# VSF1/foo_dsp_resampler

Hardware: AMD Instinct MI355X
Metric: Msamples/s, 44.1k->96k float32 'Best' (input channel-samples) (higher is better)
Workload: dtype f64; 1 GPU; BASELINE configs[1]: 44.1k->96k 2ch float32 Best; 256 independent 2-channel streams on this GPU, 481689 frames per push, device-resident in/out (RRX_flow_device); streams_per_gpu=256, frames_per_push=481689, channels=2, chain=dft->poly

## Files before the change

foo_dsp_resampler_amd/csrc/fused_fast.hip:

```cpp
#include "fft_device.hpp"
#include "fifo_device.hpp"
#include "kernels.hpp"

#include <algorithm>
#include <atomic>
#include <cstdlib>
#include <cstdio>
#include <type_traits>

namespace rsmp {

namespace {
typedef unsigned int rsmp_v2u __attribute__((ext_vector_type(2)));
typedef unsigned int rsmp_v4u __attribute__((ext_vector_type(4)));
template <typename E> struct Frame;
template <> struct Frame<float> {
  typedef float2 P;
  static __device__ __forceinline__ double in(float s) { return (double)s; }
  static __device__ __forceinline__ float out(double y) { return (float)y; }
};
template <> struct Frame<double> {
  typedef double2 P;
  static __device__ __forceinline__ double in(double s) { return s; }
  static __device__ __forceinline__ double out(double y) { return y; }
};
template <> struct Frame<short> {
  typedef short2 P;
  static __device__ __forceinline__ double in(short s) { return pcm_in(s); }
  static __device__ __forceinline__ short out(double y) { return pcm_out16(y); }
};
template <> struct Frame<int> {
  typedef int2 P;
  static __device__ __forceinline__ double in(int s) { return pcm_in(s); }
  static __device__ __forceinline__ int out(double y) { return pcm_out32(y); }
};
__device__ __forceinline__ double2 load_g(const double2 *p) { return *p; }
constexpr int kPad = 32;
constexpr int kSA = kFusedSA, kSB0 = kFusedSB0;
}

template <int LOG2P, int KS, bool OUT64, bool SPLIT, bool OGEN, bool TWO = false, typename E = float>
__device__ __forceinline__ void fused_fast_body(const FusedArgs &a, const FastIo &io)
{
  typedef Frame<E> Fr;
  typedef typename Fr::P E2;
  const E *const io_in = static_cast<const E *>(io.in), *const io_in_ring = static_cast<const E *>(io.in_ring);
  E *const io_out = static_cast<E *>(io.out), *const io_out_ring = static_cast<E *>(io.out_ring);
  static_assert(!TWO || SPLIT, "two rounds from registers: sub-blocked form only");
  static_assert(!SPLIT || LOG2P == 12, "sub-blocked form: 4096-point components");
  static_assert(!OGEN || (SPLIT && !OUT64), "generic float output exists for the sub-blocked form only");
  constexpr int LOG2N = 12, N = 1 << LOG2N, P = 1 << LOG2P;
  constexpr int T = N / 16, TF = P / 16;
  extern __shared__ __attribute__((aligned(16))) double lds[];

  const int tid = threadIdx.x;
  const int npairs = a.d.C >> 1;
  int bl, pair;
  if (!item_map(blockIdx.x, a.d.nblocks, npairs, a.d.hp, bl, pair)) return;
  const long long B = a.d.B0 + bl;
  const int hp = io.nch >> 1, strm = pair / hp, pin = pair - strm * hp;
  SubBlock sb = {0, 0, 0, 0};
  long long e0_split = 0;
  if constexpr (SPLIT) {
    const int kr = bl / a.d.nsub;
    sb = sub_block(bl - kr * a.d.nsub, a.d.V, a.d.Vs, a.d.Pref);
    e0_split = (a.d.Bref0 + kr) * a.d.q + sb.win;
  }
  const int V = SPLIT ? sb.len : a.d.V;
  const bool fwd_active = tid < TF;
  const double2 *__restrict__ Gp = a.d.G;
  double2 *smp = reinterpret_cast<double2 *>(lds) + kPad;
  const int nm1 = a.n - 1;

#ifdef RSMP_STAMPS_BUILD
  const bool stamping = a.stamps && (blockIdx.x & 63) == 5;
  unsigned long long tstamp = stamping ? __builtin_readcyclecounter() : 0;
#define RSMP_STAMP(slot)                                          \
  if (stamping) {                                                  \
    const unsigned long long now = __builtin_readcyclecounter();  \
    if (tid == 0) atomicAdd(a.stamps + (slot), now - tstamp);      \
    tstamp = now;                                                  \
  }
#else
#define RSMP_STAMP(slot)
#endif

  constexpr bool FWD8 = LOG2P == LOG2N - 1;
  constexpr int NLD = FWD8 ? 8 : 16, TL = FWD8 ? T : TF;
  c64 v[16];
  c64 u8[8];
  c64 z0[SPLIT ? 16 : 1];
  double2 wf[FWD8 ? fft8_tw_regs(LOG2P) : 1];
  if constexpr (FWD8) fft8_tw_load<LOG2P>(wf, tid, a.d.tw_fwd8);
  {
    const long long e0 = SPLIT ? e0_split : B * a.d.q;
    const bool ld_active = FWD8 || fwd_active;
    if (SPLIT && io.in_unaligned) {
      const E *pe = io_in + strm * io.in_stream_stride + 2 * pin, *pr = io_in_ring + strm * io.in_ring_stream_stride + 2 * pin;
#pragma unroll
      for (int s = 0; s < NLD; ++s) {
        const long long e = e0 + tid + s * TL;
        const E *f = e >= io.in_abs0 ? pe + (e - io.in_abs0) * io.nch : pr + (e & io.in_ring_mask) * io.nch;
        v[s] = {Fr::in(f[0]), Fr::in(f[1])};
      }
    } else
    if (e0 >= io.in_abs0) {
      const E2 *p2 = reinterpret_cast<const E2 *>(io_in + strm * io.in_stream_stride + (e0 - io.in_abs0) * io.nch + 2 * pin);
      if (ld_active) {
#pragma unroll
        for (int s = 0; s < NLD; ++s) {
          const E2 f = p2[(unsigned)((tid + s * TL) * hp)];
          (FWD8 ? u8[s & 7] : v[s]) = {Fr::in(f.x), Fr::in(f.y)};
        }
      }
    } else if (ld_active) {
      const E *pe = io_in + strm * io.in_stream_stride + 2 * pin, *pr = io_in_ring + strm * io.in_ring_stream_stride + 2 * pin;
#pragma unroll
      for (int s = 0; s < NLD; ++s) {
        const long long e = e0 + tid + s * TL;
        const E2 f = *reinterpret_cast<const E2 *>(e >= io.in_abs0 ? pe + (e - io.in_abs0) * io.nch : pr + (e & io.in_ring_mask) * io.nch);
        (FWD8 ? u8[s & 7] : v[s]) = {Fr::in(f.x), Fr::in(f.y)};
      }
    }
  }
  RSMP_STAMP(0)
  if constexpr (FWD8) {
    double2 g[16];
    fft8_regs_pre<LOG2P, -1>(u8, tid, wf, lds, [&](int p) {
      if (p == 1) {
#pragma unroll
        for (int s = 0; s < 16; ++s) g[s] = load_g(Gp + (unsigned)(tid + s * T));
      }
    });
    RSMP_STAMP(1)
#pragma unroll
    for (int s = 0; s < 16; ++s) v[s] = cmul(u8[s & 7], c64{g[s].x, g[s].y});
    __syncthreads();
  } else {
  fft_regs<LOG2P, -1, LOG2P == LOG2N ? 2 : 0, kPfFwd>(v, tid, fwd_active, a.d.tw_fwd, lds);
  RSMP_STAMP(1)
  if constexpr (LOG2P < LOG2N) {
    double2 g[16];
#pragma unroll
    for (int s = 0; s < 16; ++s) g[s] = load_g(Gp + tid + s * T);
    double2 *l2 = reinterpret_cast<double2 *>(lds);
    if (fwd_active) {
#pragma unroll
      for (int u = 0; u < 8; ++u) l2[tid + u * TF] = make_double2(v[2 * u + 1].x, v[2 * u + 1].y);
    }
    __syncthreads();
    c64 z[8];
    if (fwd_active) {
#pragma unroll
      for (int u = 0; u < 8; ++u) z[u] = v[2 * u];
    } else {
#pragma unroll
      for (int u = 0; u < 8; ++u) {
        const double2 q = l2[tid - TF + u * TF];
        z[u] = {q.x, q.y};
      }
    }
#pragma unroll
    for (int s = 0; s < 16; ++s) v[s] = cmul(z[s & 7], c64{g[s].x, g[s].y});
    __syncthreads();
  } else if constexpr (SPLIT) {
    c64 xs[16];
#pragma unroll
    for (int s = 0; s < 16; ++s) {
      xs[s] = v[s];
      const double2 g = load_g(Gp + tid + s * T);
      v[s] = cmul(xs[s], c64{g.x, g.y});
    }
    fft_regs<LOG2N, +1, 2, kPfInv>(v, tid, true, a.d.tw_inv, lds);
    double2 g1[16];
#pragma unroll
    for (int s = 0; s < 16; ++s) g1[s] = load_g(Gp + N + tid + s * T);
#pragma unroll
    for (int s = 0; s < 16; ++s) {
      z0[s] = v[s];
      v[s] = cmul(xs[s], c64{g1[s].x, g1[s].y});
    }
    __syncthreads();
    fft_regs<LOG2N, +1, 2, kPfInv>(v, tid, true, a.d.tw_inv, lds);
  } else {
#pragma unroll
    for (int s = 0; s < 16; ++s) {
      const double2 g = load_g(Gp + tid + s * T);
      v[s] = cmul(v[s], c64{g.x, g.y});
    }
  }
  }
  RSMP_STAMP(2)
  if constexpr (!SPLIT) fft_regs<LOG2N, +1, 2, kPfInv>(v, tid, true, a.d.tw_inv, lds);
  RSMP_STAMP(3)

  const int ca = 2 * pair, cb = ca + 1;
  {
    const int slot = (int)(B & a.seam_mask);
    double *seamA = a.seam + ((long long)(slot * (a.d.C + 1) + ca) * 2) * 32;
    double *seamB = a.seam + ((long long)(slot * (a.d.C + 1) + cb) * 2) * 32;
    if constexpr (SPLIT && TWO) {
      __syncthreads();
#pragma unroll
      for (int s = 0; s <= kSplitSA; ++s) {
        const int n = 2 * (tid + s * T);
        if (n < V && (s < kSplitSA || tid < kPad / 2)) {
          smp[n] = make_double2(z0[s].x, z0[s].y);
          smp[n + 1] = make_double2(v[s].x, v[s].y);
        }
      }
      if (tid < kPad) {
        smp[tid - kPad] = make_double2(0.0, 0.0);
        if (V < kSplitRaEnd + kPad) smp[V + tid] = make_double2(0.0, 0.0);
      }
      (void)seamA; (void)seamB;
    } else if constexpr (SPLIT) {
      __syncthreads();
#pragma unroll
      for (int s = 0; s < 16; ++s) {
        const int n = 2 * (tid + s * T - sb.shift);
        if (n >= 0 && n < V) {
          smp[n] = make_double2(z0[s].x, z0[s].y);
          smp[n + 1] = make_double2(v[s].x, v[s].y);
        }
      }
      if (tid < kPad) {
        smp[tid - kPad] = make_double2(0.0, 0.0);
        smp[V + tid] = make_double2(0.0, 0.0);
      }
      (void)seamA; (void)seamB;
    } else {
#pragma unroll
    for (int s = 0; s <= kSA; ++s) {
      const int n = tid + s * T;
      const bool whole = (s + 1) * T <= V;
      if (s < kSA ? (whole || n < V) : (tid < kPad && n < V)) smp[n] = make_double2(v[s].x, v[s].y);
    }
    if (tid < nm1) {
      seamA[tid] = v[0].x;
      seamB[tid] = v[0].y;
    }
    if (tid < kPad) {
      smp[tid - kPad] = make_double2(0.0, 0.0);
      if (V < kSA * T + kPad) smp[V + tid] = make_double2(0.0, 0.0);
    }
    }
  }
  __syncthreads();
  if constexpr (SPLIT) {
    if (tid < nm1) {
      const int slot = (int)(B & a.seam_mask);
      const double2 t = smp[tid];
      a.seam[((long long)(slot * (a.d.C + 1) + ca) * 2) * 32 + tid] = t.x;
      a.seam[((long long)(slot * (a.d.C + 1) + cb) * 2) * 32 + tid] = t.y;
    }
  }
  const int tail0 = V - nm1;
  auto store_tail = [&](const double2 *img, int n0) {
    if (tid < nm1) {
      const int slot = (int)(B & a.seam_mask);
      const double2 t = img[tail0 + tid - n0];
      a.seam[((long long)(slot * (a.d.C + 1) + ca) * 2 + 1) * 32 + tid] = t.x;
      a.seam[((long long)(slot * (a.d.C + 1) + cb) * 2 + 1) * 32 + tid] = t.y;
    }
  };
  const bool tail_in_b = TWO ? tail0 >= kSplitRbStart : (!SPLIT && tail0 >= kSB0 * T);
  if (!tail_in_b) store_tail(smp, 0);
  RSMP_STAMP(4)

  const FusedBlock fb = a.blk[bl];
  const int lane = tid & 63, wave = __builtin_amdgcn_readfirstlane(tid >> 6);
  const int hi = lane >> 4, bq = (lane >> 2) & 3, jq = lane & 3;
  const int pl = a.polyL, step = a.step;
  const int frame_bytes = io.nch * (int)sizeof(E);
  char *const obytes = (OUT64 || OGEN) ? nullptr
                            : reinterpret_cast<char *>(io_out + strm * io.out_stream_stride + (a.out_offset2 + fb.i_lo - io.out_abs0) * io.nch + 2 * pin);
  const long long oabs0 = a.out_offset2 + fb.i_lo;
  E *const oext = OGEN ? io_out + strm * io.out_stream_stride + 2 * pin : nullptr;
  E *const oring = OGEN ? io_out_ring + strm * io.out_ring_stream_stride + 2 * pin : nullptr;
  const unsigned o64 = OUT64 ? (unsigned)((a.out_offset2 + fb.i_lo) & io.out64_mask) : 0u;
  const unsigned m64 = (unsigned)io.out64_mask;
  __amdgpu_buffer_rsrc_t orsrcA, orsrcB;
  if constexpr (OUT64) {
    double *ra = io.out64 + (long long)(2 * pair) * io.out64_chan_stride;
    orsrcA = __builtin_amdgcn_make_buffer_rsrc(ra, 0, (int)((io.out64_mask + 1) * 8), 0x00020000);
    orsrcB = __builtin_amdgcn_make_buffer_rsrc(ra + io.out64_chan_stride, 0, (int)((io.out64_mask + 1) * 8), 0x00020000);
  }
  const int rloc = 4 * bq + hi;
  const int ngrp = a.NGRP;
  const double2 *const cfm_lane = a.cfm2 + lane;
  const int *const qtab_lane = a.qtab + bq;

  const FusedWalk fw = fused_walk(fb, ngrp);
  auto poly_round = [&](int kb, int ke, const double2 *xs, int li_lo, int li_hi) {
    if (ke <= kb) return;
    const WalkRound wr = walk_round(fw, fb.K, kb, ke, ngrp);
    const int t0 = (wr.nt * wave) >> 2, t1 = (wr.nt * (wave + 1)) >> 2;
    if (t0 >= t1) return;
    int g, pc;
    walk_seek(wr, t0, g, pc);
    g = __builtin_amdgcn_readfirstlane(g);
    int p0 = __builtin_amdgcn_readfirstlane(walk_p0(fw, g));
    pc = __builtin_amdgcn_readfirstlane(4 * pc + p0);
    int pend = __builtin_amdgcn_readfirstlane(p0 + 4 * walk_ncs(fw, fb.K, kb, ke, g));
    const int lane_li = walk_lane_li(fb, kb, hi, jq, step);
    const int lane_ib = walk_lane_ib(fb, kb, jq, rloc, pl);
    const int cnt = walk_round_cnt(fb, fw, ke, pl);
    const __amdgpu_buffer_rsrc_t orsrc =
        __builtin_amdgcn_make_buffer_rsrc(obytes, 0, (!OUT64 && !OGEN && cnt > 0) ? (cnt - 1) * frame_bytes + 2 * (int)sizeof(E) : 0, 0x00020000);
    const int lane_off0 = __mul24(lane_ib, frame_bytes);
    const bool lane_dead_last = 16 * (ngrp - 1) + rloc >= pl;

    double cc[KS], cn[KS];
    double qcd = 0.0, qnd = 0.0;
    int qci = 0, qni = 0;
    auto load_tile = [&](int gg, double (&c_)[KS], double &qd_, int &qi_) {
      constexpr int KSP = (KS + 1) / 2;
      const double2 *cp = cfm_lane + gg * (KSP * 64);
#pragma unroll
      for (int s2 = 0; s2 < KSP; ++s2) {
        const double2 d = cp[s2 * 64];
        c_[2 * s2] = d.x;
        if (2 * s2 + 1 < KS) c_[2 * s2 + 1] = d.y;
        else qd_ = d.y;
      }
      if (!(KS & 1)) qi_ = qtab_lane[gg * 4];
    };
    auto qof = [&](double qd_, int qi_) { return (KS & 1) ? (int)qd_ : qi_; };
    load_tile(g, cc, qcd, qci);
    load_tile(min(g + 1, ngrp - 1), cn, qnd, qni);

    double2 x0[KS], x1[KS];
    auto fill = [&](double2 (&x)[KS], int q, int pstep) {
      const int li = max(li_lo, min(li_hi, q + pstep * step));
      const double2 *xp = xs + li;
#pragma unroll
      for (int s = 0; s < KS; ++s) x[s] = xp[4 * s];
    };
    int qc = qof(qcd, qci) + lane_li;
    fill(x0, qc, pc);

    int left = t1 - t0;
    auto tile = [&](const double2 (&xc)[KS], double2 (&xn)[KS]) {
      int wrap;
      asm("s_lshr_b32 %0, %1, 31" : "=s"(wrap) : "s"(pend - 8 - pc));
      const int gnext = g + wrap;
      int pnext = pc + 4, pend_next = pend;
      if (wrap != 0 && left > 1) {
        if constexpr (KS & 1) asm volatile("v_cvt_i32_f64 %0, %1" : "=v"(qc) : "v"(qnd));
        else asm volatile("v_mov_b32 %0, %1" : "=v"(qc) : "v"(qni));
        qc += lane_li;
        if (gnext == wr.b1 || gnext == wr.b2) {
          p0 = __builtin_amdgcn_readfirstlane(walk_p0(fw, gnext));
          pend_next = __builtin_amdgcn_readfirstlane(p0 + 4 * walk_ncs(fw, fb.K, kb, ke, gnext));
        }
        pnext = p0;
      }
      fill(xn, qc, left > 1 ? pnext : pc);
      double accA = 0.0, accB = 0.0;
#pragma unroll
      for (int s = 0; s < KS; ++s) {
        accA = __builtin_amdgcn_mfma_f64_4x4x4f64(cc[s], xc[s].x, accA, 0, 0, 0);
        accB = __builtin_amdgcn_mfma_f64_4x4x4f64(cc[s], xc[s].y, accB, 0, 0, 0);
      }
      (void)x0;
      const int ib = lane_ib + 16 * g + pc * pl;
      if constexpr (OGEN) {
        if ((unsigned)ib < (unsigned)cnt && 16 * g + rloc < pl) {
          const long long A = oabs0 + ib;
          E *const p = (A >= io.out_abs0 && A < io.out_end) ? oext + (A - io.out_abs0) * io.nch : oring + (A & io.out_ring_mask) * io.nch;
          if (io.out_unaligned) {
            p[0] = Fr::out(accA);
            p[1] = Fr::out(accB);
          } else
            *reinterpret_cast<E2 *>(p) = E2{Fr::out(accA), Fr::out(accB)};
        }
      } else if constexpr (OUT64) {
        const bool ok = (unsigned)ib < (unsigned)cnt && 16 * g + rloc < pl;
        const unsigned off = ok ? ((o64 + (unsigned)ib) & m64) * 8u : 0xffffffffu;
        const rsmp_v2u da = {(unsigned)__double2loint(accA), (unsigned)__double2hiint(accA)};
        const rsmp_v2u db = {(unsigned)__double2loint(accB), (unsigned)__double2hiint(accB)};
        __builtin_amdgcn_raw_buffer_store_b64(da, orsrcA, (int)off, 0, 0);
        __builtin_amdgcn_raw_buffer_store_b64(db, orsrcB, (int)off, 0, 0);
      } else {
        unsigned off = (unsigned)(lane_off0 + (16 * g + pc * pl) * frame_bytes);
        if (g == ngrp - 1 && (pl & 15)) {
          off = lane_dead_last ? 0xffffffffu : off;
          asm volatile("" : "+v"(off));
        }
        if constexpr (sizeof(E) == 8) {
          const rsmp_v4u d = {(unsigned)__double2loint(accA), (unsigned)__double2hiint(accA), (unsigned)__double2loint(accB),
                              (unsigned)__double2hiint(accB)};
          __builtin_amdgcn_raw_buffer_store_b128(d, orsrc, (int)off, 0, 0);
        } else if constexpr (sizeof(E) == 2) {
          __builtin_amdgcn_raw_buffer_store_b32(pcm_pack16(accA, accB), orsrc, (int)off, 0, 0);
        } else if constexpr (std::is_same<E, int>::value) {
          const rsmp_v2u d = {(unsigned)pcm_out32(accA), (unsigned)pcm_out32(accB)};
          __builtin_amdgcn_raw_buffer_store_b64(d, orsrc, (int)off, 0, 0);
        } else {
          const rsmp_v2u d = {__float_as_uint((float)accA), __float_as_uint((float)accB)};
          __builtin_amdgcn_raw_buffer_store_b64(d, orsrc, (int)off, 0, 0);
        }
      }
      if (wrap != 0 && left > 1) {
#pragma unroll
        for (int s = 0; s < KS; ++s) asm volatile("v_mov_b64 %0, %1" : "=v"(cc[s]) : "v"(cn[s]));
        __builtin_amdgcn_sched_barrier(0);
        load_tile(min(gnext + 1, ngrp - 1), cn, qnd, qni);
      }
      g = gnext;
      pc = pnext;
      pend = pend_next;
      --left;
    };
    while (true) {
      tile(x0, x1);
      if (left == 0) break;
      tile(x1, x0);
      if (left == 0) break;
    }
  };

  const bool run = fb.cnt > 0;
  if constexpr (SPLIT && TWO) {
    if (run) poly_round(0, fw.ka, smp, -kPad, min(V, kSplitRaEnd) + kPad - 4 * KS);
    __syncthreads();
    {
      double2 *l2 = reinterpret_cast<double2 *>(lds);
#pragma unroll
      for (int s = kSplitSB0; s < 16; ++s) {
        const int n = 2 * (tid + s * T);
        if (n < V) {
          l2[n - kSplitRbStart] = make_double2(z0[s].x, z0[s].y);
          l2[n + 1 - kSplitRbStart] = make_double2(v[s].x, v[s].y);
        }
      }
      if (tid < kPad && V > kSplitRbStart) l2[V - kSplitRbStart + tid] = make_double2(0.0, 0.0);
    }
    __syncthreads();
    if (tail_in_b) store_tail(reinterpret_cast<const double2 *>(lds), kSplitRbStart);
    if (run && fw.ka < fb.K) poly_round(fw.ka, fb.K, reinterpret_cast<const double2 *>(lds) - kSplitRbStart, kSplitRbStart, V + kPad - 4 * KS);
    return;
  } else if constexpr (SPLIT) {
    if (run) poly_round(0, fb.K, smp, -kPad, V + kPad - 4 * KS);
    return;
  }
  if (run) poly_round(0, fw.ka, smp, -kPad, min(V, kSA * T) + kPad - 4 * KS);
  RSMP_STAMP(6)
  __syncthreads();
  {
    double2 *l2 = reinterpret_cast<double2 *>(lds);
#pragma unroll
    for (int s = kSB0; s < 16; ++s) {
      const int n = tid + s * T;
      if (n < V) l2[n - kSB0 * T] = make_double2(v[s].x, v[s].y);
    }
    if (tid < kPad && V > kSB0 * T) l2[V - kSB0 * T + tid] = make_double2(0.0, 0.0);
  }
  __syncthreads();
  if (tail_in_b) store_tail(reinterpret_cast<const double2 *>(lds), kSB0 * T);
  if (run && fw.ka < fb.K) poly_round(fw.ka, fb.K, reinterpret_cast<const double2 *>(lds) - kSB0 * T, kSB0 * T, V + kPad - 4 * KS);
  RSMP_STAMP(5)
#ifdef RSMP_STAMPS_BUILD
  if (stamping && tid == 0) atomicAdd(a.stamps + 7, 1ull);
#endif
#undef RSMP_STAMP
}

template <int LOG2P, int KS, bool OUT64>
__global__ __launch_bounds__(256, kFusedWaves) void fused_fast_kernel(FusedArgs a, FastIo io)
{
  fused_fast_body<LOG2P, KS, OUT64, false, false>(a, io);
}
template <int KS, int OMODE>
__global__ __launch_bounds__(256, 2) void fused_split_kernel(FusedArgs a, FastIo io)
{
  fused_fast_body<12, KS, OMODE == 1, true, OMODE == 2>(a, io);
}
template <int KS, int OMODE>
__global__ __launch_bounds__(256, 2) void fused_split2_kernel(FusedArgs a, FastIo io)
{
  fused_fast_body<12, KS, OMODE == 1, true, OMODE == 2, true>(a, io);
}

template <int LOG2P, int KS, bool OUT64>
__global__ __launch_bounds__(256, kFusedWaves) void fused_fast_dio_kernel(FusedArgs a, FastIo io)
{
  fused_fast_body<LOG2P, KS, OUT64, false, false, false, double>(a, io);
}
template <int KS, int OMODE>
__global__ __launch_bounds__(256, 2) void fused_split_dio_kernel(FusedArgs a, FastIo io)
{
  fused_fast_body<12, KS, OMODE == 1, true, OMODE == 2, false, double>(a, io);
}
template <int KS, int OMODE>
__global__ __launch_bounds__(256, 2) void fused_split2_dio_kernel(FusedArgs a, FastIo io)
{
  fused_fast_body<12, KS, OMODE == 1, true, OMODE == 2, true, double>(a, io);
}

#define RSMP_PCM_KERNELS(tag, E)                                                                                          \
  template <int LOG2P, int KS, bool OUT64>                                                                                \
  __global__ __launch_bounds__(256, kFusedWaves) void fused_fast_##tag##_kernel(FusedArgs a, FastIo io)                  \
  {                                                                                                                       \
    fused_fast_body<LOG2P, KS, OUT64, false, false, false, E>(a, io);                                                     \
  }                                                                                                                       \
  template <int KS, int OMODE> __global__ __launch_bounds__(256, 2) void fused_split_##tag##_kernel(FusedArgs a, FastIo io) \
  {                                                                                                                       \
    fused_fast_body<12, KS, OMODE == 1, true, OMODE == 2, false, E>(a, io);                                               \
  }                                                                                                                       \
  template <int KS, int OMODE> __global__ __launch_bounds__(256, 2) void fused_split2_##tag##_kernel(FusedArgs a, FastIo io) \
  {                                                                                                                       \
    fused_fast_body<12, KS, OMODE == 1, true, OMODE == 2, true, E>(a, io);                                                \
  }
RSMP_PCM_KERNELS(s16, short)
RSMP_PCM_KERNELS(s32, int)
#undef RSMP_PCM_KERNELS

typedef void (*FastKernel)(FusedArgs, FastIo);

template <int LOG2P, int KS, bool OUT64> static hipError_t launch_fast_t(const FusedArgs &a, const FastIo &io, hipStream_t st)
{
  constexpr int N = 4096;
  size_t lds_bytes = 8 * size_t(fft_lds_doubles_halves(12));
  if (LOG2P < 12) lds_bytes = std::max(lds_bytes, 8 * size_t(std::max(fft_lds_doubles(LOG2P), fft8_lds_doubles(LOG2P))));
  lds_bytes = std::max(lds_bytes, size_t(kPad + kSA * (N / 16) + kPad) * 16);
  static DynLdsOnce attr[4];
  static const FastKernel fns[4] = {&fused_fast_kernel<LOG2P, KS, OUT64>, &fused_fast_dio_kernel<LOG2P, KS, OUT64>,
                                    &fused_fast_s16_kernel<LOG2P, KS, OUT64>, &fused_fast_s32_kernel<LOG2P, KS, OUT64>};
  if (io.dio < 0 || io.dio > 3) return hipErrorInvalidValue;
  if (hipError_t e = attr[io.dio].set(reinterpret_cast<const void *>(fns[io.dio]), int(lds_bytes)); e != hipSuccess) return e;
  FusedArgs b = a;
  b.d.hp = io.nch >= 4 ? io.nch / 2 : 0;
  dim3 grid(item_grid(a.d.nblocks, a.d.C / 2, b.d.hp)), block(N / 16);
  hipLaunchKernelGGL(fns[io.dio], grid, block, lds_bytes, st, b, io);
  return hipGetLastError();
}

template <int KS, int OMODE, bool TWO> static hipError_t launch_split_t(const FusedArgs &a, const FastIo &io, hipStream_t st)
{
  const size_t lds_max = std::max(size_t(8) * fft_lds_doubles_halves(12), size_t(kPad + (TWO ? kSplitRaEnd : kSplitVsMax) + kPad) * 16);
  const size_t lds_bytes = TWO ? lds_max : std::max(size_t(8) * fft_lds_doubles_halves(12), size_t(kPad + a.d.Vs + kPad) * 16);
  static DynLdsOnce attr[4];
  static const FastKernel fns[4] = {
      TWO ? &fused_split2_kernel<KS, OMODE> : &fused_split_kernel<KS, OMODE>, TWO ? &fused_split2_dio_kernel<KS, OMODE> : &fused_split_dio_kernel<KS, OMODE>,
      TWO ? &fused_split2_s16_kernel<KS, OMODE> : &fused_split_s16_kernel<KS, OMODE>, TWO ? &fused_split2_s32_kernel<KS, OMODE> : &fused_split_s32_kernel<KS, OMODE>};
  if (io.dio < 0 || io.dio > 3) return hipErrorInvalidValue;
  if (hipError_t e = attr[io.dio].set(reinterpret_cast<const void *>(fns[io.dio]), int(lds_max)); e != hipSuccess) return e;
  FusedArgs b = a;
  b.d.hp = io.nch >= 4 ? io.nch / 2 : 0;
  dim3 grid(item_grid(a.d.nblocks, a.d.C / 2, b.d.hp)), block(256);
  hipLaunchKernelGGL(fns[io.dio], grid, block, lds_bytes, st, b, io);
  return hipGetLastError();
}

bool fused_split_two_supported(int V, int taps, int ksteps, int qb_spread)
{
  return !knobs().no_split2 && !(V & 1) && V == 8192 - (taps - 1) && V > kSplitVsMax && V - kSplitRbStart + kPad <= kSplitRaEnd + kPad &&
         qb_spread + 4 * ksteps + 4 <= kSplitRaEnd - kSplitRbStart + kPad && ksteps >= 7 && ksteps <= 9;
}

bool fused_split_supported(int log2n, int L, int ksteps)
{
  return !knobs().no_fast && !knobs().no_split && L == 2 && log2n >= 13 && log2n <= 15 && ksteps >= 7 && ksteps <= 9;
}

hipError_t launch_fused_split(int omode, const FusedArgs &a, const FastIo &io, hipStream_t st, const char **kname)
{
  if (a.d.two) {
    if (a.d.nsub != 1 || a.d.Vs != a.d.V || a.d.Pref != 4096 || a.d.V <= kSplitVsMax || a.d.V > 8192 || (a.d.V & 1)) return hipErrorInvalidValue;
  } else if (a.d.Vs > kSplitVsMax) return hipErrorInvalidValue;
  if (a.d.nsub < 1 || a.d.Vs < 64 || (a.d.Vs & 1) || (a.d.V & 1) || a.d.nblocks % a.d.nsub || omode < 0 || omode > 2 ||
      (omode == 1 ? !io.out64 : omode == 2 ? !io.out_ring : !io.out) ||
      (a.d.Pref != 4096 && a.d.Pref != 8192 && a.d.Pref != 16384) || a.d.nsub * a.d.Vs < a.d.V || (a.d.nsub - 1) * a.d.Vs >= a.d.V || (io.nch & 1))
    return hipErrorInvalidValue;
  for (int i = 0; i < a.d.nsub; ++i) {
    const SubBlock sb = sub_block(i, a.d.V, a.d.Vs, a.d.Pref);
    const int ov = 2 * a.d.Pref - a.d.V;
    if (sb.win < 0 || sb.shift < 0 || sb.shift + sb.len / 2 + (ov + 1) / 2 > 4096 || (sb.len & 1) || sb.win + 4096 > a.d.Pref) return hipErrorInvalidValue;
  }
#define RSMP_IO_NAME(fmt, head, tail) \
  ((fmt) == 1 ? head "_dio_" tail : (fmt) == 2 ? head "_s16_" tail : (fmt) == 3 ? head "_s32_" tail : head "_" tail)
#define RSMP_SPLIT_CASE(ks, om)                                                        \
  if (a.KS == ks && omode == om && !a.d.two) {                                         \
    if (kname) *kname = RSMP_IO_NAME(io.dio, "rsmp::fused_split", "kernel<" #ks ", " #om ">");  \
    return launch_split_t<ks, om, false>(a, io, st);                                   \
  }                                                                                    \
  if (a.KS == ks && omode == om && a.d.two) {                                          \
    if (kname) *kname = RSMP_IO_NAME(io.dio, "rsmp::fused_split2", "kernel<" #ks ", " #om ">"); \
    return launch_split_t<ks, om, true>(a, io, st);                                    \
  }
  RSMP_SPLIT_CASE(7, 0) RSMP_SPLIT_CASE(7, 1) RSMP_SPLIT_CASE(7, 2) RSMP_SPLIT_CASE(8, 0) RSMP_SPLIT_CASE(8, 1) RSMP_SPLIT_CASE(8, 2)
  RSMP_SPLIT_CASE(9, 0) RSMP_SPLIT_CASE(9, 1) RSMP_SPLIT_CASE(9, 2)
#undef RSMP_SPLIT_CASE
  return hipErrorInvalidValue;
}

size_t fused_walk_enumerate(const FusedPrepArgs &p, int k, long long *head, int *slots, size_t cap)
{
  const FusedBlock fb = fused_block_info(p, k);
  const int pl = p.polyL, step = p.step, ngrp = (pl + 15) >> 4;
  const FusedWalk fw = fused_walk(fb, ngrp);
  const FusedWalk uni = {0, ngrp, fb.KA};
  const long long h[13] = {fb.i_lo, fb.cnt, fb.K, fb.KA, fb.walk < 0, fw.g_lo, fw.g_hi, fw.ka,
                           fb.cnt > 0 ? fused_walk_tiles(fw, fb.K, ngrp) : 0, fb.cnt > 0 ? fused_walk_tiles(uni, fb.K, ngrp) : 0,
                           fb.irel_lo, fb.base_li, ngrp};
  for (int i = 0; i < 13; ++i) head[i] = h[i];
  size_t n = 0;
  if (fb.cnt <= 0) return 0;
  for (int round = 0; round < 2; ++round) {
    const int kb = round ? fw.ka : 0, ke = round ? fb.K : fw.ka;
    if (ke <= kb) continue;
    const WalkRound wr = walk_round(fw, fb.K, kb, ke, ngrp);
    const int cnt = walk_round_cnt(fb, fw, ke, pl);
    for (int wave = 0; wave < 4; ++wave) {
      const int t0 = (wr.nt * wave) >> 2, t1 = (wr.nt * (wave + 1)) >> 2;
      if (t0 >= t1) continue;
      int g, c;
      walk_seek(wr, t0, g, c);
      int pc = 4 * c + walk_p0(fw, g), pend = walk_p0(fw, g) + 4 * walk_ncs(fw, fb.K, kb, ke, g);
      for (int left = t1 - t0; left > 0; --left) {
        for (int lane = 0; lane < 64; ++lane) {
          const int hi = lane >> 4, bq = (lane >> 2) & 3, jq = lane & 3, rloc = 4 * bq + hi;
          const long long a0 = p.at0 + (long long)(16 * g + 4 * bq) * step;
          const int li = walk_lane_li(fb, kb, hi, jq, step) + int(a0 / pl) + pc * step;
          const int ib = walk_lane_ib(fb, kb, jq, rloc, pl) + 16 * g + pc * pl;
          if (n < cap) {
            int *o = slots + 7 * n;
            o[0] = round, o[1] = g, o[2] = (pc - walk_p0(fw, g)) >> 2, o[3] = lane, o[4] = ib;
            o[5] = ib >= 0 && ib < cnt && 16 * g + rloc < pl;
            o[6] = li;
          }
          ++n;
        }
        if (pc + 4 == pend) {
          ++g;
          pc = walk_p0(fw, g);
          pend = pc + 4 * walk_ncs(fw, fb.K, kb, ke, g);
        } else
          pc += 4;
      }
    }
  }
  return n;
}

bool fused_fast_supported(int log2n, int log2p, int ksteps)
{
  return !knobs().no_fast && log2n == 12 && (log2p == 11 || log2p == 12) && (ksteps == 7 || ksteps == 8);
}

#define RSMP_FAST_CASE(p, ks)                                                                        \
  if (log2p == p && a.KS == ks) {                                                                    \
    if (kname) *kname = io.out64 ? RSMP_IO_NAME(io.dio, "rsmp::fused_fast", "kernel<" #p ", " #ks ", true>") \
                                 : RSMP_IO_NAME(io.dio, "rsmp::fused_fast", "kernel<" #p ", " #ks ", false>"); \
    return io.out64 ? launch_fast_t<p, ks, true>(a, io, st) : launch_fast_t<p, ks, false>(a, io, st); \
  }

hipError_t launch_fused_fast(int log2p, const FusedArgs &a, const FastIo &io, hipStream_t st, const char **kname)
{
  RSMP_FAST_CASE(11, 7) RSMP_FAST_CASE(12, 7) RSMP_FAST_CASE(11, 8) RSMP_FAST_CASE(12, 8)
  return hipErrorInvalidValue;
}

}
```

Measured before the change: 127,700 Msamples/s.

## Prefetch polyphase coefficient tiles before LDS staging and hand off across rounds

Restructures the non-split fused kernel so the polyphase walk setup and first coefficient tile loads for both LDS rounds are issued before the FFT results are written to LDS and the barrier runs. The last prefetch of round A loads round B's first tile, so round B starts without a fresh global load. The goal is to hide coefficient fetch latency behind the LDS staging and syncs. The cost is more live registers across the staging section, which can lower occupancy, plus more complex control flow for the handoff.

Result: no change. 128,600 Msamples/s (median of 6 runs) (+0.8%).

```diff
diff --git a/foo_dsp_resampler_amd/csrc/fused_fast.hip b/foo_dsp_resampler_amd/csrc/fused_fast.hip
--- a/foo_dsp_resampler_amd/csrc/fused_fast.hip
+++ b/foo_dsp_resampler_amd/csrc/fused_fast.hip
@@ -123,6 +123,9 @@
       }
     }
   }
+  const FusedBlock fb = a.blk[bl];
+  const int ngrp = a.NGRP;
+  const FusedWalk fw = fused_walk(fb, ngrp);
   RSMP_STAMP(0)
   if constexpr (FWD8) {
     double2 g[16];
@@ -193,82 +196,12 @@
   RSMP_STAMP(2)
   if constexpr (!SPLIT) fft_regs<LOG2N, +1, 2, kPfInv>(v, tid, true, a.d.tw_inv, lds);
   RSMP_STAMP(3)
-
-  const int ca = 2 * pair, cb = ca + 1;
-  {
-    const int slot = (int)(B & a.seam_mask);
-    double *seamA = a.seam + ((long long)(slot * (a.d.C + 1) + ca) * 2) * 32;
-    double *seamB = a.seam + ((long long)(slot * (a.d.C + 1) + cb) * 2) * 32;
-    if constexpr (SPLIT && TWO) {
-      __syncthreads();
-#pragma unroll
-      for (int s = 0; s <= kSplitSA; ++s) {
-        const int n = 2 * (tid + s * T);
-        if (n < V && (s < kSplitSA || tid < kPad / 2)) {
-          smp[n] = make_double2(z0[s].x, z0[s].y);
-          smp[n + 1] = make_double2(v[s].x, v[s].y);
-        }
-      }
-      if (tid < kPad) {
-        smp[tid - kPad] = make_double2(0.0, 0.0);
-        if (V < kSplitRaEnd + kPad) smp[V + tid] = make_double2(0.0, 0.0);
-      }
-      (void)seamA; (void)seamB;
-    } else if constexpr (SPLIT) {
-      __syncthreads();
-#pragma unroll
-      for (int s = 0; s < 16; ++s) {
-        const int n = 2 * (tid + s * T - sb.shift);
-        if (n >= 0 && n < V) {
-          smp[n] = make_double2(z0[s].x, z0[s].y);
-          smp[n + 1] = make_double2(v[s].x, v[s].y);
-        }
-      }
-      if (tid < kPad) {
-        smp[tid - kPad] = make_double2(0.0, 0.0);
-        smp[V + tid] = make_double2(0.0, 0.0);
-      }
-      (void)seamA; (void)seamB;
-    } else {
-#pragma unroll
-    for (int s = 0; s <= kSA; ++s) {
-      const int n = tid + s * T;
-      const bool whole = (s + 1) * T <= V;
-      if (s < kSA ? (whole || n < V) : (tid < kPad && n < V)) smp[n] = make_double2(v[s].x, v[s].y);
-    }
-    if (tid < nm1) {
-      seamA[tid] = v[0].x;
-      seamB[tid] = v[0].y;
-    }
-    if (tid < kPad) {
-      smp[tid - kPad] = make_double2(0.0, 0.0);
-      if (V < kSA * T + kPad) smp[V + tid] = make_double2(0.0, 0.0);
-    }
-    }
-  }
-  __syncthreads();
-  if constexpr (SPLIT) {
-    if (tid < nm1) {
-      const int slot = (int)(B & a.seam_mask);
-      const double2 t = smp[tid];
-      a.seam[((long long)(slot * (a.d.C + 1) + ca) * 2) * 32 + tid] = t.x;
-      a.seam[((long long)(slot * (a.d.C + 1) + cb) * 2) * 32 + tid] = t.y;
-    }
-  }
-  const int tail0 = V - nm1;
-  auto store_tail = [&](const double2 *img, int n0) {
-    if (tid < nm1) {
-      const int slot = (int)(B & a.seam_mask);
-      const double2 t = img[tail0 + tid - n0];
-      a.seam[((long long)(slot * (a.d.C + 1) + ca) * 2 + 1) * 32 + tid] = t.x;
-      a.seam[((long long)(slot * (a.d.C + 1) + cb) * 2 + 1) * 32 + tid] = t.y;
-    }
-  };
-  const bool tail_in_b = TWO ? tail0 >= kSplitRbStart : (!SPLIT && tail0 >= kSB0 * T);
-  if (!tail_in_b) store_tail(smp, 0);
-  RSMP_STAMP(4)
-
-  const FusedBlock fb = a.blk[bl];
+  if constexpr (!SPLIT) {
+#pragma unroll
+    for (int s = 0; s < 16; ++s) asm volatile("" : "+v"(v[s].x), "+v"(v[s].y));
+    __builtin_amdgcn_sched_barrier(0);
+  }
+
   const int lane = tid & 63, wave = __builtin_amdgcn_readfirstlane(tid >> 6);
   const int hi = lane >> 4, bq = (lane >> 2) & 3, jq = lane & 3;
   const int pl = a.polyL, step = a.step;
@@ -287,49 +220,76 @@
     orsrcB = __builtin_amdgcn_make_buffer_rsrc(ra + io.out64_chan_stride, 0, (int)((io.out64_mask + 1) * 8), 0x00020000);
   }
   const int rloc = 4 * bq + hi;
-  const int ngrp = a.NGRP;
   const double2 *const cfm_lane = a.cfm2 + lane;
   const int *const qtab_lane = a.qtab + bq;
 
-  const FusedWalk fw = fused_walk(fb, ngrp);
-  auto poly_round = [&](int kb, int ke, const double2 *xs, int li_lo, int li_hi) {
-    if (ke <= kb) return;
+  struct RoundWalk { int kb, ke, b1, b2, g, pc, p0, pend, left; };
+  auto round_walk = [&](int kb, int ke) {
+    RoundWalk w = {kb, ke, 0, 0, 0, 0, 0, 0, 0};
+    if (ke <= kb) return w;
     const WalkRound wr = walk_round(fw, fb.K, kb, ke, ngrp);
     const int t0 = (wr.nt * wave) >> 2, t1 = (wr.nt * (wave + 1)) >> 2;
-    if (t0 >= t1) return;
-    int g, pc;
-    walk_seek(wr, t0, g, pc);
-    g = __builtin_amdgcn_readfirstlane(g);
-    int p0 = __builtin_amdgcn_readfirstlane(walk_p0(fw, g));
-    pc = __builtin_amdgcn_readfirstlane(4 * pc + p0);
-    int pend = __builtin_amdgcn_readfirstlane(p0 + 4 * walk_ncs(fw, fb.K, kb, ke, g));
-    const int lane_li = walk_lane_li(fb, kb, hi, jq, step);
-    const int lane_ib = walk_lane_ib(fb, kb, jq, rloc, pl);
-    const int cnt = walk_round_cnt(fb, fw, ke, pl);
-    const __amdgpu_buffer_rsrc_t orsrc =
-        __builtin_amdgcn_make_buffer_rsrc(obytes, 0, (!OUT64 && !OGEN && cnt > 0) ? (cnt - 1) * frame_bytes + 2 * (int)sizeof(E) : 0, 0x00020000);
-    const int lane_off0 = __mul24(lane_ib, frame_bytes);
-    const bool lane_dead_last = 16 * (ngrp - 1) + rloc >= pl;
-
-    double cc[KS], cn[KS];
-    double qcd = 0.0, qnd = 0.0;
-    int qci = 0, qni = 0;
-    auto load_tile = [&](int gg, double (&c_)[KS], double &qd_, int &qi_) {
-      constexpr int KSP = (KS + 1) / 2;
-      const double2 *cp = cfm_lane + gg * (KSP * 64);
-#pragma unroll
-      for (int s2 = 0; s2 < KSP; ++s2) {
-        const double2 d = cp[s2 * 64];
-        c_[2 * s2] = d.x;
-        if (2 * s2 + 1 < KS) c_[2 * s2 + 1] = d.y;
-        else qd_ = d.y;
-      }
-      if (!(KS & 1)) qi_ = qtab_lane[gg * 4];
-    };
-    auto qof = [&](double qd_, int qi_) { return (KS & 1) ? (int)qd_ : qi_; };
-    load_tile(g, cc, qcd, qci);
-    load_tile(min(g + 1, ngrp - 1), cn, qnd, qni);
-
+    if (t0 >= t1) return w;
+    int g_, c_;
+    walk_seek(wr, t0, g_, c_);
+    w.b1 = wr.b1, w.b2 = wr.b2;
+    w.g = __builtin_amdgcn_readfirstlane(g_);
+    w.p0 = __builtin_amdgcn_readfirstlane(walk_p0(fw, w.g));
+    w.pc = __builtin_amdgcn_readfirstlane(4 * c_ + w.p0);
+    w.pend = __builtin_amdgcn_readfirstlane(w.p0 + 4 * walk_ncs(fw, fb.K, kb, ke, w.g));
+    w.left = __builtin_amdgcn_readfirstlane(t1 - t0);
+    return w;
+  };
+  int rkb = 0, rke = 0, rb1 = 0, rb2 = 0;
+  int lane_li = 0, lane_ib = 0, lane_off0 = 0, cnt = 0;
+  __amdgpu_buffer_rsrc_t orsrc;
+  const bool lane_dead_last = 16 * (ngrp - 1) + rloc >= pl;
+  auto round_begin = [&](const RoundWalk &w) {
+    rkb = w.kb, rke = w.ke, rb1 = w.b1, rb2 = w.b2;
+    lane_li = walk_lane_li(fb, rkb, hi, jq, step);
+    lane_ib = walk_lane_ib(fb, rkb, jq, rloc, pl);
+    cnt = walk_round_cnt(fb, fw, rke, pl);
+    orsrc = __builtin_amdgcn_make_buffer_rsrc(obytes, 0, (!OUT64 && !OGEN && cnt > 0) ? (cnt - 1) * frame_bytes + 2 * (int)sizeof(E) : 0, 0x00020000);
+    lane_off0 = __mul24(lane_ib, frame_bytes);
+  };
+
+  double cc[KS], cn[KS];
+  double qcd = 0.0, qnd = 0.0;
+  int qci = 0, qni = 0;
+  auto load_tile = [&](int gg, double (&c_)[KS], double &qd_, int &qi_) {
+    constexpr int KSP = (KS + 1) / 2;
+    const double2 *cp = cfm_lane + gg * (KSP * 64);
+#pragma unroll
+    for (int s2 = 0; s2 < KSP; ++s2) {
+      const double2 d = cp[s2 * 64];
+      c_[2 * s2] = d.x;
+      if (2 * s2 + 1 < KS) c_[2 * s2 + 1] = d.y;
+      else qd_ = d.y;
+    }
+    if (!(KS & 1)) qi_ = qtab_lane[gg * 4];
+  };
+  auto qof = [&](double qd_, int qi_) { return (KS & 1) ? (int)qd_ : qi_; };
+  int g_hand = -1;
+  auto round_tiles = [&](const RoundWalk &w) {
+    load_tile(w.g, cc, qcd, qci);
+    int gl = min(w.g + 1, ngrp - 1);
+    if (g_hand >= 0 && 4 * w.left <= w.pend - w.pc) gl = g_hand;
+    load_tile(gl, cn, qnd, qni);
+  };
+
+  auto round_run = [&](const RoundWalk &w, const double2 *xs, int li_lo, int li_hi, int handed) {
+    if (w.left == 0) return;
+    int g = w.g, pc = w.pc, p0 = w.p0, pend = w.pend, left = w.left;
+    int qc;
+    if (handed != 0) {
+      if constexpr (KS & 1) asm volatile("v_cvt_i32_f64 %0, %1" : "=v"(qc) : "v"(qnd));
+      else asm volatile("v_mov_b32 %0, %1" : "=v"(qc) : "v"(qni));
+#pragma unroll
+      for (int s = 0; s < KS; ++s) asm volatile("v_mov_b64 %0, %1" : "=v"(cc[s]) : "v"(cn[s]));
+      __builtin_amdgcn_sched_barrier(0);
+      load_tile(min(g + 1, ngrp - 1), cn, qnd, qni);
+    } else
+      qc = qof(qcd, qci);
     double2 x0[KS], x1[KS];
     auto fill = [&](double2 (&x)[KS], int q, int pstep) {
       const int li = max(li_lo, min(li_hi, q + pstep * step));
@@ -337,10 +297,9 @@
 #pragma unroll
       for (int s = 0; s < KS; ++s) x[s] = xp[4 * s];
     };
-    int qc = qof(qcd, qci) + lane_li;
+    qc += lane_li;
     fill(x0, qc, pc);
 
-    int left = t1 - t0;
     auto tile = [&](const double2 (&xc)[KS], double2 (&xn)[KS]) {
       int wrap;
       asm("s_lshr_b32 %0, %1, 31" : "=s"(wrap) : "s"(pend - 8 - pc));
@@ -350,9 +309,9 @@
         if constexpr (KS & 1) asm volatile("v_cvt_i32_f64 %0, %1" : "=v"(qc) : "v"(qnd));
         else asm volatile("v_mov_b32 %0, %1" : "=v"(qc) : "v"(qni));
         qc += lane_li;
-        if (gnext == wr.b1 || gnext == wr.b2) {
+        if (gnext == rb1 || gnext == rb2) {
           p0 = __builtin_amdgcn_readfirstlane(walk_p0(fw, gnext));
-          pend_next = __builtin_amdgcn_readfirstlane(p0 + 4 * walk_ncs(fw, fb.K, kb, ke, gnext));
+          pend_next = __builtin_amdgcn_readfirstlane(p0 + 4 * walk_ncs(fw, fb.K, rkb, rke, gnext));
         }
         pnext = p0;
       }
@@ -406,7 +365,9 @@
 #pragma unroll
         for (int s = 0; s < KS; ++s) asm volatile("v_mov_b64 %0, %1" : "=v"(cc[s]) : "v"(cn[s]));
         __builtin_amdgcn_sched_barrier(0);
-        load_tile(min(gnext + 1, ngrp - 1), cn, qnd, qni);
+        int gl = min(gnext + 1, ngrp - 1);
+        if (g_hand >= 0 && 4 * (left - 1) <= pend_next - pnext) gl = g_hand;
+        load_tile(gl, cn, qnd, qni);
       }
       g = gnext;
       pc = pnext;
@@ -420,8 +381,100 @@
       if (left == 0) break;
     }
   };
-
   const bool run = fb.cnt > 0;
+  RoundWalk wa = {}, wb = {};
+  if constexpr (!SPLIT) {
+    if (run) {
+      wa = round_walk(0, fw.ka);
+      wb = round_walk(fw.ka, fb.K);
+      if (wa.left > 0 && wb.left > 0) g_hand = wb.g;
+      round_begin(wa);
+      if (wa.left > 0) round_tiles(wa);
+    }
+  }
+
+
+  const int ca = 2 * pair, cb = ca + 1;
+  {
+    const int slot = (int)(B & a.seam_mask);
+    double *seamA = a.seam + ((long long)(slot * (a.d.C + 1) + ca) * 2) * 32;
+    double *seamB = a.seam + ((long long)(slot * (a.d.C + 1) + cb) * 2) * 32;
+    if constexpr (SPLIT && TWO) {
+      __syncthreads();
+#pragma unroll
+      for (int s = 0; s <= kSplitSA; ++s) {
+        const int n = 2 * (tid + s * T);
+        if (n < V && (s < kSplitSA || tid < kPad / 2)) {
+          smp[n] = make_double2(z0[s].x, z0[s].y);
+          smp[n + 1] = make_double2(v[s].x, v[s].y);
+        }
+      }
+      if (tid < kPad) {
+        smp[tid - kPad] = make_double2(0.0, 0.0);
+        if (V < kSplitRaEnd + kPad) smp[V + tid] = make_double2(0.0, 0.0);
+      }
+      (void)seamA; (void)seamB;
+    } else if constexpr (SPLIT) {
+      __syncthreads();
+#pragma unroll
+      for (int s = 0; s < 16; ++s) {
+        const int n = 2 * (tid + s * T - sb.shift);
+        if (n >= 0 && n < V) {
+          smp[n] = make_double2(z0[s].x, z0[s].y);
+          smp[n + 1] = make_double2(v[s].x, v[s].y);
+        }
+      }
+      if (tid < kPad) {
+        smp[tid - kPad] = make_double2(0.0, 0.0);
+        smp[V + tid] = make_double2(0.0, 0.0);
+      }
+      (void)seamA; (void)seamB;
+    } else {
+#pragma unroll
+    for (int s = 0; s <= kSA; ++s) {
+      const int n = tid + s * T;
+      const bool whole = (s + 1) * T <= V;
+      if (s < kSA ? (whole || n < V) : (tid < kPad && n < V)) smp[n] = make_double2(v[s].x, v[s].y);
+    }
+    if (tid < nm1) {
+      seamA[tid] = v[0].x;
+      seamB[tid] = v[0].y;
+    }
+    if (tid < kPad) {
+      smp[tid - kPad] = make_double2(0.0, 0.0);
+      if (V < kSA * T + kPad) smp[V + tid] = make_double2(0.0, 0.0);
+    }
+    }
+  }
+  __syncthreads();
+  if constexpr (SPLIT) {
+    if (tid < nm1) {
+      const int slot = (int)(B & a.seam_mask);
+      const double2 t = smp[tid];
+      a.seam[((long long)(slot * (a.d.C + 1) + ca) * 2) * 32 + tid] = t.x;
+      a.seam[((long long)(slot * (a.d.C + 1) + cb) * 2) * 32 + tid] = t.y;
+    }
+  }
+  const int tail0 = V - nm1;
+  auto store_tail = [&](const double2 *img, int n0) {
+    if (tid < nm1) {
+      const int slot = (int)(B & a.seam_mask);
+      const double2 t = img[tail0 + tid - n0];
+      a.seam[((long long)(slot * (a.d.C + 1) + ca) * 2 + 1) * 32 + tid] = t.x;
+      a.seam[((long long)(slot * (a.d.C + 1) + cb) * 2 + 1) * 32 + tid] = t.y;
+    }
+  };
+  const bool tail_in_b = TWO ? tail0 >= kSplitRbStart : (!SPLIT && tail0 >= kSB0 * T);
+  if (!tail_in_b) store_tail(smp, 0);
+  RSMP_STAMP(4)
+
+  auto poly_round = [&](int kb, int ke, const double2 *xs, int li_lo, int li_hi) {
+    const RoundWalk w = round_walk(kb, ke);
+    if (w.left == 0) return;
+    round_begin(w);
+    round_tiles(w);
+    round_run(w, xs, li_lo, li_hi, 0);
+  };
   if constexpr (SPLIT && TWO) {
     if (run) poly_round(0, fw.ka, smp, -kPad, min(V, kSplitRaEnd) + kPad - 4 * KS);
     __syncthreads();
@@ -445,7 +498,11 @@
     if (run) poly_round(0, fb.K, smp, -kPad, V + kPad - 4 * KS);
     return;
   }
-  if (run) poly_round(0, fw.ka, smp, -kPad, min(V, kSA * T) + kPad - 4 * KS);
+  round_run(wa, smp, -kPad, min(V, kSA * T) + kPad - 4 * KS, 0);
+  const int handed = g_hand >= 0;
+  g_hand = -1;
+  round_begin(wb);
+  if (wb.left > 0 && handed == 0) round_tiles(wb);
   RSMP_STAMP(6)
   __syncthreads();
   {
@@ -459,7 +516,7 @@
   }
   __syncthreads();
   if (tail_in_b) store_tail(reinterpret_cast<const double2 *>(lds), kSB0 * T);
-  if (run && fw.ka < fb.K) poly_round(fw.ka, fb.K, reinterpret_cast<const double2 *>(lds) - kSB0 * T, kSB0 * T, V + kPad - 4 * KS);
+  round_run(wb, reinterpret_cast<const double2 *>(lds) - kSB0 * T, kSB0 * T, V + kPad - 4 * KS, handed);
   RSMP_STAMP(5)
 #ifdef RSMP_STAMPS_BUILD
   if (stamping && tid == 0) atomicAdd(a.stamps + 7, 1ull);
```
